# cvlab-stonybrook/s-volsdf

Hardware: AMD Instinct MI355X
Metric: rendered rays/sec (1024-ray batch, 128 samples) (higher is better)
Workload: dtype f32 (every product, forward and backward, as three fp16 MFMA products of two-piece fp16 operands with f32 accumulate; activation blocks hold both pieces: float32 accuracy class); 1 GPU; configs[1]: VolOpt.train_step (forward + MVS prior lookup + loss + backward + clip/guard/Adam), train mode, fast=1: 1024 rays/GPU x 128 coarse + 98 composited samples + 2048 eikonal points, 8x256 SDF MLP + 4x256 radiance MLP; mode=train, mlp_precision=fp16x2, launch=eager launches, rays_per_gpu=1024, rays_total=1024

## Files before the change

s-volsdf_amd/csrc/svs_sampler.hip:

```cpp
#include "svs_common.h"

namespace svs {
namespace sampler {

constexpr int kCap = 768;
constexpr int kMaxNew = 128;

struct Ctl {
  int conv_flag[8];
  int active[8];
  int final_round;
};

__device__ __forceinline__ float fma32(float a, float b, float c) { return __builtin_fmaf(a, b, c); }

__device__ __forceinline__ float linspace_at(float start, float end, int n, int i) {
  const float step = (end - start) / (float)(n - 1);
  return i < n / 2 ? fma32(step, (float)i, start) : fma32(-step, (float)(n - 1 - i), end);
}

__device__ __forceinline__ float wave_cumsum(const float* in, float* out, int m, int lane) {
  const int c = (m + 63) >> 6;
  const int lo = lane * c;
  const int hi = (lo + c < m) ? lo + c : m;
  double tot = 0.0;
  for (int j = lo; j < hi; ++j) tot = tot + (double)in[j];
  double scan = tot;
#pragma unroll
  for (int d = 1; d < 64; d <<= 1) {
    const double o = __shfl_up(scan, d);
    if (lane >= d) scan = scan + o;
  }
  double off = __shfl_up(scan, 1);
  if (lane == 0) off = 0.0;
  double acc = 0.0;
  float last = 0.0f;
  for (int j = lo; j < hi; ++j) {
    acc = acc + (double)in[j];
    last = (float)(off + acc);
    out[j] = last;
  }
  const int owner = (m - 1) / c;
  return __shfl(last, owner);
}

__device__ __forceinline__ float wave_max(float v) {
#pragma unroll
  for (int d = 32; d >= 1; d >>= 1) v = __builtin_fmaxf(v, __shfl_xor(v, d));
  return v;
}

struct RayLds {
  float z[kCap];
  float sdf[kCap];
  float dists[kCap];
  float dstar[kCap];
  float t0[kCap];
  float t1[kCap];
};

__device__ __forceinline__ void compute_dstar(RayLds& L, int n, int lane) {
  for (int i = lane; i < n - 1; i += 64) {
    const float a = L.z[i + 1] - L.z[i];
    const float d0 = L.sdf[i], d1 = L.sdf[i + 1];
    const float b = __builtin_fabsf(d0), c = __builtin_fabsf(d1);
    const float a2 = a * a, b2 = b * b, c2 = c * c;
    const bool first = (a2 + b2) <= c2;
    const bool second = (a2 + c2) <= b2;
    float ds = 0.0f;
    if (first) ds = b;
    if (second) ds = c;
    const float s = ((a + b) + c) / 2.0f;
    const float area = ((s * (s - a)) * (s - b)) * (s - c);
    if (!first && !second && ((b + c) - a > 0.0f)) ds = (2.0f * __builtin_sqrtf(area)) / a;
    const float sg0 = d0 > 0.0f ? 1.0f : (d0 < 0.0f ? -1.0f : 0.0f);
    const float sg1 = d1 > 0.0f ? 1.0f : (d1 < 0.0f ? -1.0f : 0.0f);
    const float same = (sg1 * sg0 == 1.0f) ? 1.0f : 0.0f;
    L.dists[i] = a;
    L.dstar[i] = same * ds;
  }
}

__device__ __forceinline__ float error_bound(RayLds& L, int n, float beta, int lane) {
  const float four_b2 = 4.0f * (beta * beta);
  for (int i = lane; i < n; i += 64) {
    L.t0[i] = i == 0 ? 0.0f : L.dists[i - 1] * laplace_density(L.sdf[i - 1], beta);
    if (i < n - 1) L.t1[i] = (sleef_expf(-L.dstar[i] / beta) * (L.dists[i] * L.dists[i])) / four_b2;
  }
  __syncthreads();
  wave_cumsum(L.t0, L.t0, n, lane);
  wave_cumsum(L.t1, L.t1, n - 1, lane);
  __syncthreads();
  float m = -__builtin_inff();
  bool has_nan = false;
  for (int i = lane; i < n - 1; i += 64) {
    const float e = sleef_expf(L.t1[i]);
    const float bo = ((e > 1.0e6f ? 1.0e6f : e) - 1.0f) * sleef_expf(-L.t0[i]);
    has_nan |= (bo != bo);
    m = __builtin_fmaxf(m, bo);
  }
  __syncthreads();
  m = wave_max(m);
  if (__any(has_nan)) m = __builtin_nanf("");
  return m;
}

struct InitArgs {
  const float* cam; int cam_stride; const float* dirs;
  int R;
  int n_eval;
  float near, far;
  int sphere_far;
  float sphere_radius;
  const float* jitter;
  float inv_4log;
  float* samples;
  float* beta;
  float* far_out;
  Ctl* ctl;
  int group_rays;
  int max_iters;
  int* err;
};

__global__ __launch_bounds__(64) void init_kernel(InitArgs a) {
  __shared__ float zs[kMaxNew];
  __shared__ float ds[kMaxNew];
  const int r = blockIdx.x, lane = threadIdx.x;
  if (r % a.group_rays == 0 && lane < 8) {
    Ctl* c = a.ctl + r / a.group_rays;
    c->conv_flag[lane] = 0;
    c->active[lane] = (lane == 0 && a.max_iters > 0) ? 1 : 0;
    if (lane == 0) c->final_round = -1;
  }
  float far = a.far;
  if (a.sphere_far) {
    const float* o = a.cam + (size_t)r * a.cam_stride;
    const float* d = a.dirs + 3 * (size_t)r;
    const float dot = (d[0] * o[0] + d[1] * o[1]) + d[2] * o[2];
    const float nrm = norm3(o[0], o[1], o[2]);
    const float under = dot * dot - (nrm * nrm - a.sphere_radius * a.sphere_radius);
    if (under <= 0.0f) { if (lane == 0) *a.err = 1; }
    far = __builtin_fmaxf(__builtin_sqrtf(under) - dot, 0.0f);
  }
  if (lane == 0) a.far_out[r] = far;
  const int n = a.n_eval;
  for (int i = lane; i < n; i += 64) {
    const float t = linspace_at(0.0f, 1.0f, n, i);
    zs[i] = a.near * (1.0f - t) + far * t;
  }
  __syncthreads();
  if (a.jitter) {
    float znew[(kMaxNew + 63) / 64];
    int k = 0;
    for (int i = lane; i < n; i += 64, ++k) {
      const float lower = i == 0 ? zs[0] : 0.5f * (zs[i] + zs[i - 1]);
      const float upper = i == n - 1 ? zs[n - 1] : 0.5f * (zs[i + 1] + zs[i]);
      znew[k] = lower + (upper - lower) * a.jitter[(size_t)r * n + i];
    }
    __syncthreads();
    k = 0;
    for (int i = lane; i < n; i += 64, ++k) zs[i] = znew[k];
    __syncthreads();
  }
  for (int i = lane; i < n; i += 64) {
    a.samples[(size_t)r * kMaxNew + i] = zs[i];
    if (i < n - 1) { const float d = zs[i + 1] - zs[i]; ds[i] = d * d; }
  }
  __syncthreads();
  const float tot = aten_row_sum(ds, n - 1, lane);
  if (lane == 0) a.beta[r] = __builtin_sqrtf(a.inv_4log * tot);
}

struct RoundArgs {
  int R, round, max_iters;
  int n_eval, n_final, n_extra;
  const float* beta_param; float beta_min;
  float eps; int beta_iters; float add_tiny;
  float near;
  const float* far;
  float* z;
  float* sdf;
  float* beta;
  float* samples;
  const float* samples_sdf;
  Ctl* ctl;
  int group_rays;
  const float* u_final;
  const int* extra_idx;
  const int* eik_idx;
  float* z_final;
  float* z_eik;
  int* dbg_samples_idx;
  int* dbg_inds;
  float* dbg_cdf;
  float* dbg_weights;
};

__global__ __launch_bounds__(64) void round_a_kernel(RoundArgs a) {
  __shared__ RayLds L;
  const int r = blockIdx.x, lane = threadIdx.x, i_round = a.round;
  Ctl* ctl = a.ctl + r / a.group_rays;
  if (!ctl->active[i_round]) return;
  const int n_old = a.n_eval * i_round, n_new = a.n_eval, n = n_old + n_new;
  float* zrow = a.z + (size_t)r * kCap;
  float* srow = a.sdf + (size_t)r * kCap;
  for (int i = lane; i < n_old; i += 64) { L.t0[i] = zrow[i]; L.t1[i] = srow[i]; }
  for (int i = lane; i < n_new; i += 64) {
    L.dists[i] = a.samples[(size_t)r * kMaxNew + i];
    L.dstar[i] = a.samples_sdf[(size_t)r * kMaxNew + i];
  }
  __syncthreads();
  for (int e = lane; e < n; e += 64) {
    int pos;
    float zv, sv;
    if (e < n_old) {
      zv = L.t0[e]; sv = L.t1[e];
      int cnt = 0;
      for (int k = 0; k < n_new; ++k) cnt += (L.dists[k] < zv) ? 1 : 0;
      pos = e + cnt;
    } else {
      const int j = e - n_old;
      zv = L.dists[j]; sv = L.dstar[j];
      int lo = 0, hi = n_old;
      while (lo < hi) { const int mid = (lo + hi) >> 1; if (L.t0[mid] <= zv) lo = mid + 1; else hi = mid; }
      int cnt = lo;
      for (int k = 0; k < n_new; ++k) {
        const float o = L.dists[k];
        cnt += (o < zv || (o == zv && k < j)) ? 1 : 0;
      }
      pos = cnt;
    }
    L.z[pos] = zv; L.sdf[pos] = sv;
    if (a.dbg_samples_idx) a.dbg_samples_idx[(size_t)r * kCap + pos] = e;
  }
  __syncthreads();
  for (int i = lane; i < n; i += 64) { zrow[i] = L.z[i]; srow[i] = L.sdf[i]; }
  compute_dstar(L, n, lane);
  __syncthreads();

  float beta = a.beta[r];
  const float beta0 = __builtin_fabsf(*a.beta_param) + a.beta_min;
  float err = error_bound(L, n, beta0, lane);
  if (err <= a.eps) beta = beta0;
  float bmin = beta0, bmax = beta;
  for (int it = 0; it < a.beta_iters; ++it) {
    const float mid = (bmin + bmax) / 2.0f;
    err = error_bound(L, n, mid, lane);
    if (err <= a.eps) bmax = mid;
    if (err > a.eps) bmin = mid;
  }
  beta = bmax;
  if (lane == 0) {
    a.beta[r] = beta;
    if (beta > beta0) atomicOr(&ctl->conv_flag[i_round], 1);
  }
}

__device__ __forceinline__ void finalize(const RoundArgs& a, RayLds& L, int r, int n, int ns, int lane) {
  const int m = ns + a.n_extra + 2;
  for (int i = lane; i < a.n_extra + 2; i += 64) {
    float v;
    if (i == 0) v = a.near;
    else if (i == 1) v = a.far[r];
    else {
      int idx;
      if (a.extra_idx) idx = a.extra_idx[i - 2];
      else idx = (int)linspace_at(0.0f, (float)(n - 1), a.n_extra, i - 2);
      v = L.z[idx];
    }
    L.t0[ns + i] = v;
  }
  __syncthreads();
  for (int e = lane; e < m; e += 64) {
    const float v = L.t0[e];
    int cnt = 0;
    for (int k = 0; k < m; ++k) { const float o = L.t0[k]; cnt += (o < v || (o == v && k < e)) ? 1 : 0; }
    L.t1[cnt] = v;
  }
  __syncthreads();
  for (int i = lane; i < m; i += 64) a.z_final[(size_t)r * m + i] = L.t1[i];
  if (lane == 0) a.z_eik[r] = L.t1[a.eik_idx ? a.eik_idx[r] : 0];
}

__global__ __launch_bounds__(64) void round_b_kernel(RoundArgs a) {
  __shared__ RayLds L;
  const int r = blockIdx.x, lane = threadIdx.x, i_round = a.round;
  Ctl* ctl = a.ctl + r / a.group_rays;
  if (!ctl->active[i_round]) return;
  const bool upsample = ctl->conv_flag[i_round] != 0 && (i_round + 1 < a.max_iters);
  if (r % a.group_rays == 0 && lane == 0) {
    ctl->active[i_round + 1] = upsample ? 1 : 0;
    if (!upsample) ctl->final_round = i_round;
  }
  const int n = a.n_eval * (i_round + 1);
  const float* zrow = a.z + (size_t)r * kCap;
  const float* srow = a.sdf + (size_t)r * kCap;
  for (int i = lane; i < n; i += 64) { L.z[i] = zrow[i]; L.sdf[i] = srow[i]; }
  __syncthreads();
  compute_dstar(L, n, lane);
  __syncthreads();
  const float beta = a.beta[r];
  for (int i = lane; i < n; i += 64) {
    L.t0[i] = i == 0 ? 0.0f : L.dists[i - 1] * laplace_density(L.sdf[i - 1], beta);
  }
  __syncthreads();
  wave_cumsum(L.t0, L.t0, n, lane);
  __syncthreads();
  for (int i = lane; i < n; i += 64) L.t0[i] = sleef_expf(-L.t0[i]);
  __syncthreads();
  const int N = upsample ? a.n_eval : a.n_final;
  if (upsample) {
    const float four_b2 = 4.0f * (beta * beta);
    for (int i = lane; i < n - 1; i += 64)
      L.t1[i] = (sleef_expf(-L.dstar[i] / beta) * (L.dists[i] * L.dists[i])) / four_b2;
    __syncthreads();
    wave_cumsum(L.t1, L.t1, n - 1, lane);
    __syncthreads();
    for (int i = lane; i < n - 1; i += 64) {
      const float e = sleef_expf(L.t1[i]);
      L.t1[i] = ((e > 1.0e6f ? 1.0e6f : e) - 1.0f) * L.t0[i] + a.add_tiny;
    }
  } else {
    for (int i = lane; i < n - 1; i += 64) {
      const float fe = L.dists[i] * laplace_density(L.sdf[i], beta);
      const float w = (1.0f - sleef_expf(-fe)) * L.t0[i];
      L.t1[i] = w + 1e-5f;
      if (a.dbg_weights) a.dbg_weights[(size_t)r * kCap + i] = w;
    }
  }
  __syncthreads();
  const float tot = aten_row_sum(L.t1, n - 1, lane);
  __syncthreads();
  for (int i = lane; i < n - 1; i += 64) L.t1[i] = L.t1[i] / tot;
  __syncthreads();
  wave_cumsum(L.t1, L.dstar, n - 1, lane);
  __syncthreads();
  for (int i = lane; i < n; i += 64) {
    const float c = i == 0 ? 0.0f : L.dstar[i - 1];
    L.t1[i] = c;
    if (a.dbg_cdf) a.dbg_cdf[(size_t)r * kCap + i] = c;
  }
  __syncthreads();
  for (int j = lane; j < N; j += 64) {
    float u;
    if (upsample || !a.u_final) u = linspace_at(0.0f, 1.0f, N, j);
    else u = a.u_final[(size_t)r * N + j];
    int lo = 0, hi = n;
    while (lo < hi) { const int mid = (lo + hi) >> 1; if (L.t1[mid] <= u) lo = mid + 1; else hi = mid; }
    const int inds = lo;
    const int below = inds - 1 > 0 ? inds - 1 : 0;
    const int above = inds < n - 1 ? inds : n - 1;
    const float cb = L.t1[below], ca = L.t1[above];
    const float zb = L.z[below], za = L.z[above];
    float denom = ca - cb;
    if (denom < 1e-5f) denom = 1.0f;
    const float t = (u - cb) / denom;
    L.dstar[j] = zb + t * (za - zb);
    if (a.dbg_inds) a.dbg_inds[(size_t)r * kMaxNew + j] = inds;
  }
  __syncthreads();
  if (upsample) {
    for (int j = lane; j < N; j += 64) a.samples[(size_t)r * kMaxNew + j] = L.dstar[j];
  } else {
    for (int j = lane; j < N; j += 64) L.t0[j] = L.dstar[j];
    __syncthreads();
    finalize(a, L, r, n, N, lane);
  }
}

__global__ __launch_bounds__(64) void finalize0_kernel(RoundArgs a) {
  __shared__ RayLds L;
  const int r = blockIdx.x, lane = threadIdx.x;
  for (int i = lane; i < a.n_eval; i += 64) {
    const float v = a.samples[(size_t)r * kMaxNew + i];
    L.z[i] = v; L.t0[i] = v;
  }
  __syncthreads();
  finalize(a, L, r, a.n_eval, a.n_eval, lane);
}

}
}

using namespace svs;
using namespace svs::sampler;

extern "C" {

size_t svs_sampler_ctl_bytes(int n_rays, int group_rays) {
  const int g = group_rays > 0 ? group_rays : (n_rays > 0 ? n_rays : 1);
  return (size_t)((n_rays + g - 1) / g) * sizeof(Ctl);
}
int svs_sampler_ctl_stride(void) { return (int)(sizeof(Ctl) / sizeof(int)); }
int svs_sampler_cap(void) { return kCap; }
int svs_sampler_max_new(void) { return kMaxNew; }

int svs_sampler_init(const float* cam, int cam_stride, const float* dirs, int n_rays, int n_eval, float near_, float far_,
                     int sphere_far, float sphere_radius, const float* jitter, float inv_4log, int max_iters,
                     float* samples, float* beta, float* far_out, void* ctl, int group_rays, int* err_flag,
                     void* hip_stream) {
  if (group_rays <= 0) group_rays = n_rays;
  if (!cam || !dirs || !samples || !beta || !far_out || !ctl || !err_flag || n_rays <= 0) {
    set_error("svs_sampler_init: null/invalid argument"); return SVS_EINVAL;
  }
  if (n_eval < 2 || n_eval > kMaxNew || max_iters < 0 || max_iters > 7 || n_eval * (max_iters > 0 ? max_iters : 1) > kCap) {
    set_error("svs_sampler_init: n_eval=%d max_iters=%d exceed the kernel limits (%d new / %d bins)", n_eval, max_iters, kMaxNew, kCap);
    return SVS_ESHAPE;
  }
  InitArgs a{cam, cam_stride, dirs, n_rays, n_eval, near_, far_, sphere_far, sphere_radius, jitter, inv_4log,
             samples, beta, far_out, (Ctl*)ctl, group_rays, max_iters, err_flag};
  init_kernel<<<n_rays, 64, 0, (hipStream_t)hip_stream>>>(a);
  return check_launch("svs_sampler_init");
}

int svs_sampler_round(int phase, int n_rays, int round, int max_iters, int n_eval, int n_final, int n_extra,
                      const float* beta_param, float beta_min, float eps, int beta_iters, float add_tiny, float near_,
                      const float* far_,
                      float* z, float* sdf, float* beta, float* samples, const float* samples_sdf, void* ctl,
                      int group_rays, const float* u_final, const int* extra_idx, const int* eik_idx, float* z_final, float* z_eik,
                      int* dbg_samples_idx, int* dbg_inds, float* dbg_cdf, float* dbg_weights, void* hip_stream) {
  if (!beta_param || !far_ || !z || !sdf || !beta || !samples || !ctl || !z_final || !z_eik || n_rays <= 0 || round < 0 || round > 6) {
    set_error("svs_sampler_round: null/invalid argument"); return SVS_EINVAL;
  }
  if (group_rays <= 0) group_rays = n_rays;
  if (n_final > kMaxNew || n_final + n_extra + 2 > kCap || n_eval + n_extra + 2 > kCap) {
    set_error("svs_sampler_round: sample counts exceed kernel limits"); return SVS_ESHAPE;
  }
  RoundArgs a{n_rays, round, max_iters, n_eval, n_final, n_extra, beta_param, beta_min, eps, beta_iters, add_tiny, near_, far_,
              z, sdf, beta, samples, samples_sdf, (Ctl*)ctl, group_rays, u_final, extra_idx, eik_idx, z_final, z_eik,
              dbg_samples_idx, dbg_inds, dbg_cdf, dbg_weights};
  hipStream_t s = (hipStream_t)hip_stream;
  if (phase == 0) {
    if (!samples_sdf) { set_error("svs_sampler_round: round A needs samples_sdf"); return SVS_EINVAL; }
    round_a_kernel<<<n_rays, 64, 0, s>>>(a);
  } else if (phase == 1) {
    round_b_kernel<<<n_rays, 64, 0, s>>>(a);
  } else {
    finalize0_kernel<<<n_rays, 64, 0, s>>>(a);
  }
  return check_launch("svs_sampler_round");
}

__global__ void selftest_exp_kernel(const float* x, float* y_exp, float* y_expm1, int n) {
  const int i = blockIdx.x * blockDim.x + threadIdx.x;
  if (i < n) { y_exp[i] = sleef_expf(x[i]); y_expm1[i] = sleef_expm1f(x[i]); }
}
__global__ void selftest_arith_kernel(const float* a, const float* b, float* q, float* s, int n) {
  const int i = blockIdx.x * blockDim.x + threadIdx.x;
  if (i < n) { q[i] = a[i] / b[i]; s[i] = __builtin_sqrtf(__builtin_fabsf(a[i])); }
}
__global__ __launch_bounds__(64) void selftest_cumsum_kernel(const float* x, float* y, float* tot, int m) {
  __shared__ float buf[kCap];
  const int lane = threadIdx.x;
  for (int i = lane; i < m; i += 64) buf[i] = x[(size_t)blockIdx.x * m + i];
  __syncthreads();
  const float t = wave_cumsum(buf, buf, m, lane);
  __syncthreads();
  for (int i = lane; i < m; i += 64) y[(size_t)blockIdx.x * m + i] = buf[i];
  if (lane == 0) tot[blockIdx.x] = t;
}

__global__ __launch_bounds__(64) void selftest_rowsum_kernel(const float* x, float* tot, int m) {
  extern __shared__ float rowbuf[];
  const int lane = threadIdx.x;
  for (int i = lane; i < m; i += 64) rowbuf[i] = x[(size_t)blockIdx.x * m + i];
  __syncthreads();
  const float t = aten_row_sum(rowbuf, m, lane);
  if (lane == 0) tot[blockIdx.x] = t;
}

int svs_selftest_rowsum(const float* x, float* tot, int rows, int m, void* hip_stream) {
  if (m < 1 || m > 16000) { set_error("svs_selftest_rowsum: m out of range (1..16000)"); return SVS_ESHAPE; }
  selftest_rowsum_kernel<<<rows, 64, (size_t)m * sizeof(float), (hipStream_t)hip_stream>>>(x, tot, m);
  return check_launch("svs_selftest_rowsum");
}
int svs_selftest_exp(const float* x, float* y_exp, float* y_expm1, int n, void* hip_stream) {
  selftest_exp_kernel<<<(n + 255) / 256, 256, 0, (hipStream_t)hip_stream>>>(x, y_exp, y_expm1, n);
  return check_launch("svs_selftest_exp");
}
int svs_selftest_arith(const float* a, const float* b, float* q, float* s, int n, void* hip_stream) {
  selftest_arith_kernel<<<(n + 255) / 256, 256, 0, (hipStream_t)hip_stream>>>(a, b, q, s, n);
  return check_launch("svs_selftest_arith");
}
int svs_selftest_cumsum(const float* x, float* y, float* tot, int rows, int m, void* hip_stream) {
  if (m < 1 || m > kCap) { set_error("svs_selftest_cumsum: m out of range"); return SVS_ESHAPE; }
  selftest_cumsum_kernel<<<rows, 64, 0, (hipStream_t)hip_stream>>>(x, y, tot, m);
  return check_launch("svs_selftest_cumsum");
}

}
```

s-volsdf_amd/svs_hip/ops.py:

```python
import ctypes
import os

import torch

from . import lib as _lib


def _ptr(t):
    if t is None:
        return None
    assert t.is_cuda and t.is_contiguous(), "device-resident contiguous tensors only"
    return t.data_ptr()


_raw_stream = getattr(torch._C, "_cuda_getCurrentRawStream", None)


def _stream():
    if _raw_stream is not None:
        return _raw_stream(torch.cuda.current_device())
    return torch.cuda.current_stream().cuda_stream


def _f32(t):
# ... 355 lines not shown
        cam, dirs, z = _f32(cam).reshape(3), _f32(dirs), _f32(z)
        R, S = z.shape
        dev = z.device
    V = len(views)
    ver = lambda t: (id(t), getattr(t, "_version", 0))
    key = tuple((ver(v["K"]), ver(v["c2w"]), v["cost"].data_ptr(), v["cost"].shape,
                 (v["z_mvs"].data_ptr(), v["z_mvs"].shape) if "z_mvs" in v else (v["z_near"].data_ptr(), v["z_far"].data_ptr()))
                for v in views)
    hit = _LOOKUP_CONSTS.get(key)
    if hit is None:
        vp = (ctypes.c_float * (17 * V))()
        dims = (ctypes.c_int * (3 * V))()
        keep, cost_p, near_p, far_p = [], [], [], []
        copied = False
        for j, v in enumerate(views):
            K, c2w = _host_f32(v["K"]), _host_f32(v["c2w"])
            vals = [K[0, 0], K[1, 1], K[0, 2], K[1, 2], K[0, 1]] + [c2w[i, k] for i in range(3) for k in range(4)]
            for k, x in enumerate(vals):
                vp[17 * j + k] = float(x)
            cost = _f32(v["cost"]).reshape(v["cost"].shape[-3:])
            if "z_mvs" in v:
                zm = v["z_mvs"].reshape(v["z_mvs"].shape[-3:])
                zn, zf = _f32(zm[0]), _f32(zm[-1])
                copied = copied or zn.data_ptr() != zm[0].data_ptr() or zf.data_ptr() != zm[-1].data_ptr()
            else:
                zn, zf = _f32(v["z_near"]), _f32(v["z_far"])
                copied = copied or zn.data_ptr() != v["z_near"].data_ptr() or zf.data_ptr() != v["z_far"].data_ptr()
            keep += [cost, zn, zf, v["K"], v["c2w"], v["cost"], v.get("z_mvs"), v.get("z_near"), v.get("z_far")]
            copied = copied or cost.data_ptr() != v["cost"].data_ptr()
            cost_p.append(cost); near_p.append(zn); far_p.append(zf)
            dims[3 * j], dims[3 * j + 1], dims[3 * j + 2] = cost.shape
        if len(_LOOKUP_CONSTS) >= 4:
            _LOOKUP_CONSTS.clear()
        hit = (vp, dims, _ptr_array(cost_p), _ptr_array(near_p), _ptr_array(far_p), keep)
        if not copied:
            _LOOKUP_CONSTS[key] = hit
    vp, dims, cost_arr, near_arr, far_arr, _ = hit
    pj = torch.empty(R, S, device=dev)
    pi = torch.empty(R, S, device=dev)
    valid = torch.empty(R, S, dtype=torch.uint8, device=dev)
    _lib.check(L.svs_cost_lookup(_ptr(xyz), _ptr(cam), _ptr(dirs), _ptr(z), S, R * S, V, int(same_view),
                                 int(bool(inverse_depth)), float(img_res[1]), float(img_res[0]), vp,
                                 cost_arr, near_arr, far_arr, dims, _ptr(pj), _ptr(pi),
                                 _ptr(valid), _ptr(same_view_dev), _stream()), "svs_cost_lookup")
    return pj, pi, valid.view(torch.bool)


def loss_fwd_bwd(rgb_values, rgb_target, weights, depth_values, grad_theta=None, pi=None, pj=None, *, rgb_weight=1.0,
                 eikonal_weight=0.1, mvs_weight=0.0, sparse_weight=0.0, gce=1.0, confi=0.0, annealed=False,
                 anneal_sparse=0.0, norm=None, anneal_dev=None, grad_theta_out=None):
    L = _lib.load()
    rgb_values, rgb_target = _f32(rgb_values).reshape(-1, 3), _f32(rgb_target).reshape(-1, 3)
    weights, depth_values = _f32(weights), _f32(depth_values).reshape(-1)
    R, S = weights.shape
    dev = weights.device
    gt = _f32(grad_theta) if grad_theta is not None else None
    n_eik = gt.shape[0] if gt is not None else 0
    pi_, pj_ = (_f32(pi), _f32(pj)) if pi is not None else (None, None)
    losses = torch.empty(5, device=dev)
    d_rgb = torch.empty(R, 3, device=dev)
    d_gt = None
    if n_eik:
        ok = (grad_theta_out is not None and grad_theta_out.is_cuda and grad_theta_out.dtype == torch.float32
              and tuple(grad_theta_out.shape) == (n_eik, 3) and grad_theta_out.is_contiguous())
        d_gt = grad_theta_out if ok else torch.empty(n_eik, 3, device=dev)
    d_w = torch.empty(R, S, device=dev)
    d_dep = torch.empty(R, 1, device=dev)
    ws = torch.empty(L.svs_loss_workspace_bytes(R, n_eik) // 8, dtype=torch.float64, device=dev)
    _lib.check(L.svs_loss(R, S, n_eik, _ptr(rgb_values), _ptr(rgb_target), _ptr(gt), _ptr(weights), _ptr(pi_), _ptr(pj_),
                          _ptr(depth_values), float(rgb_weight), float(eikonal_weight), float(mvs_weight),
                          float(sparse_weight), float(gce), float(confi), int(bool(annealed)), float(anneal_sparse),
                          int(norm[0]) if norm else 0, int(norm[1]) if norm else 0, _ptr(losses), _ptr(d_rgb), _ptr(d_gt), _ptr(d_w), _ptr(d_dep), _ptr(ws),
                          _ptr(anneal_dev), _stream()), "svs_loss")
    return losses, dict(rgb_values=d_rgb, grad_theta=d_gt, weights=d_w, depth_values=d_dep)


class SamplerWorkspace:

    def __init__(self, R, device, group_rays=None):
        L = _lib.load()
        self.R = R
        self.group_rays = int(group_rays) if group_rays else R
        self.cap, self.max_new = L.svs_sampler_cap(), L.svs_sampler_max_new()
        f = lambda *s: torch.empty(*s, device=device)
        self.z, self.sdf = f(R, self.cap), f(R, self.cap)
        self.beta, self.far = f(R), f(R)
        self.samples, self.samples_sdf = f(R, self.max_new), f(R, self.max_new)
        self.ctl = torch.zeros(L.svs_sampler_ctl_bytes(R, self.group_rays) // 4, dtype=torch.int32, device=device)
        self.ctl_stride = L.svs_sampler_ctl_stride()
        self.err = torch.zeros(1, dtype=torch.int32, device=device)


def sample_rays(packed, cam, dirs, beta_param, *, beta_min=1e-4, near, scene_bounding_sphere, sphere_scale, sdf_clamp_radius,
                N_samples=64, N_samples_eval=128, N_samples_extra=32, eps=0.1, beta_iters=10, max_total_iters=5,
                fast=-1, training=False, inverse_sphere_bg=False, add_tiny=0.0, inv_4log=None, rng=None,
                workspace=None, debug=None, sdf_override=None):
    L = _lib.load()
    cam, dirs = _f32(cam), _f32(dirs)
    R = dirs.shape[0]
    dev = dirs.device
    ws = workspace or SamplerWorkspace(R, dev)
    assert ws.R == R
    rng = rng or {}
    if not torch.is_tensor(beta_param):
        beta_param = torch.tensor(float(beta_param), device=dev)
    beta_param = _f32(beta_param).reshape(1)
    max_iters = fast if fast >= 0 else max_total_iters
    if training and max_iters > 1 and "perm" in rng:
        raise NotImplementedError("train-mode extras for more than one round need the bin count on the host")
    if inv_4log is None:
        inv_4log = float(1.0 / (4.0 * torch.log(torch.tensor(eps + 1.0))))
    cam_stride = 0 if cam.numel() == 3 else 3
    far = 2.0 * scene_bounding_sphere
    jitter = _f32(rng["jitter"]) if training and "jitter" in rng else None
    _lib.check(L.svs_sampler_init(_ptr(cam), cam_stride, _ptr(dirs), R, N_samples_eval, float(near), float(far),
                                  int(inverse_sphere_bg), float(scene_bounding_sphere), _ptr(jitter), float(inv_4log),
                                  max_iters, _ptr(ws.samples), _ptr(ws.beta), _ptr(ws.far), _ptr(ws.ctl), ws.group_rays,
                                  _ptr(ws.err), _stream()), "svs_sampler_init")
    n_out = (N_samples if max_iters > 0 else N_samples_eval) + N_samples_extra + 2
    z_final = torch.empty(R, n_out, device=dev)
    z_eik = torch.empty(R, 1, device=dev)
    u_final = _f32(rng["u"]) if training and "u" in rng else None
    extra_idx = rng["perm"].to(torch.int32).contiguous() if training and "perm" in rng else None
    eik_idx = rng["eik_idx"].to(torch.int32).contiguous() if training and "eik_idx" in rng else None

    def call(phase, i, dbg):
        _lib.check(L.svs_sampler_round(phase, R, i, max_iters, N_samples_eval, N_samples, N_samples_extra, _ptr(beta_param),
                                       float(beta_min), float(eps), beta_iters, float(add_tiny), float(near), _ptr(ws.far), _ptr(ws.z),
                                       _ptr(ws.sdf), _ptr(ws.beta), _ptr(ws.samples), _ptr(ws.samples_sdf), _ptr(ws.ctl),
                                       ws.group_rays, _ptr(u_final), _ptr(extra_idx), _ptr(eik_idx), _ptr(z_final), _ptr(z_eik),
                                       _ptr(dbg.get("samples_idx")), _ptr(dbg.get("inds")), _ptr(dbg.get("cdf")),
                                       _ptr(dbg.get("weights")), _stream()), "svs_sampler_round")

    if max_iters == 0:
        call(2, 0, {})
        return z_final, z_eik
    src = PointSource(cam=cam, dirs=dirs, z=ws.samples[:, :N_samples_eval]) if N_samples_eval == ws.max_new else None
    for i in range(max_iters):
        dbg = {}
        if debug is not None:
            dbg = dict(samples_idx=torch.full((R, ws.cap), -1, dtype=torch.int32, device=dev),
                       inds=torch.full((R, ws.max_new), -1, dtype=torch.int32, device=dev),
                       cdf=torch.zeros(R, ws.cap, device=dev), weights=torch.zeros(R, ws.cap, device=dev))
            debug.setdefault("rounds", []).append(dbg)
        if sdf_override is not None:
            if i < len(sdf_override):
                ws.samples_sdf[:, :N_samples_eval].copy_(sdf_override[i])
        else:
            if src is None:
                raise NotImplementedError("N_samples_eval must equal the kernel's row stride (128)")
            gate = ws.ctl.data_ptr() + 4 * (8 + i)
            sdf_vals(packed, src, sdf_clamp_radius, sphere_scale, out=ws.samples_sdf, gate=gate,
                     gate_points=ws.group_rays * N_samples_eval, gate_stride=ws.ctl_stride)
        call(0, i, dbg)
        call(1, i, dbg)
        if debug is not None:
            dbg["z"] = ws.z.clone(); dbg["sdf"] = ws.sdf.clone(); dbg["beta"] = ws.beta.clone()
            dbg["samples"] = ws.samples.clone(); dbg["ctl"] = ws.ctl.clone()
    return z_final, z_eik
```

s-volsdf_amd/svs_hip/trainer.py:

```python
import ctypes

import os

import torch

from . import lib as _lib
from . import ops
from .ops import _ptr, _stream


class FlatParams:

    def __init__(self, params):
        self.params = [p for p in params]
        dev = self.params[0].device
        n = sum(p.numel() for p in self.params)
        self.flat = torch.empty(n, device=dev)
        self.grad = torch.zeros(n, device=dev)
        off = 0
        for p in self.params:
            k = p.numel()
            self.flat[off:off + k].copy_(p.data.reshape(-1))
            p.data = self.flat[off:off + k].view(p.shape)
            p.grad = self.grad[off:off + k].view(p.shape)
            off += k
        self.n = n

    def views(self, buf):
        out, off = [], 0
        for p in self.params:
            out.append(buf[off:off + p.numel()].view(p.shape))
            off += p.numel()
        return out


class FusedAdam:

    def __init__(self, params, lr=5e-4, betas=(0.9, 0.999), eps=1e-8, max_norm=1.0):
        self.fp = params if isinstance(params, FlatParams) else FlatParams(list(params))
        self.lr, self.betas, self.eps, self.max_norm = lr, betas, eps, max_norm
        dev = self.fp.flat.device
        self.exp_avg = torch.zeros_like(self.fp.flat)
        self.exp_avg_sq = torch.zeros_like(self.fp.flat)
        L = _lib.load()
        self.ws = torch.empty(L.svs_adam_workspace_bytes() // 4, dtype=torch.int32, device=dev)
        self.info = torch.zeros(2, device=dev)
        self.step_count = 0
        self.step_dev = None

    def zero_grad(self, set_to_none=False):
        self.fp.grad.zero_()

    def step(self):
        L = _lib.load()
        self.step_count += 1
        _lib.check(L.svs_clip_guard_adam(_ptr(self.fp.flat), _ptr(self.fp.grad), _ptr(self.exp_avg), _ptr(self.exp_avg_sq),
                                         self.fp.n, self.step_count, _ptr(self.step_dev) if self.step_dev is not None else None,
                                         float(self.max_norm), float(self.lr), float(self.betas[0]), float(self.betas[1]),
                                         float(self.eps), _ptr(self.ws), _ptr(self.info), _stream()), "svs_clip_guard_adam")

    def state_dict(self):
        return {"step": self.step_count, "exp_avg": self.exp_avg, "exp_avg_sq": self.exp_avg_sq}

    def load_state_dict(self, sd):
        self.step_count = int(sd["step"])
        self.exp_avg.copy_(sd["exp_avg"]); self.exp_avg_sq.copy_(sd["exp_avg_sq"])


def shard_rays(uv, rank, world):
    R = uv.shape[1]
    if R % world:
        raise ValueError(f"{R} rays do not shard over {world} ranks")
    k = R // world
    return uv[:, rank * k:(rank + 1) * k]


def allreduce_flat_grad(flat_grad, world):
    import torch.distributed as dist
    if world > 1 or (dist.is_available() and dist.is_initialized()):
        dist.all_reduce(flat_grad, op=dist.ReduceOp.SUM)
    return flat_grad


def data_parallel(world):
    import torch.distributed as dist
    return world > 1 or (dist.is_available() and dist.is_initialized())


def grad_buckets(n_sdf, n):
    return [(n_sdf, n), (0, n_sdf)]


def allreduce_range(flat_grad, lo, hi, async_op=False):
    import torch.distributed as dist
    return dist.all_reduce(flat_grad[lo:hi], op=dist.ReduceOp.SUM, async_op=async_op)


_DP_BUCKETS = os.environ.get("SVS_DP_BUCKETS", "1") == "1"


class _GroupedOutputs(dict):

    def __init__(self, results):
        super().__init__()
        self._parts = [r[1] for r in results]

    def __missing__(self, key):
        vals = [p[key] for p in self._parts]
        self[key] = torch.cat(vals, 0) if torch.is_tensor(vals[0]) and vals[0].dim() > 0 else vals[0]
        return self[key]

    def __contains__(self, key):
        return key in self._parts[0]

    def keys(self):
        return self._parts[0].keys()


class _ValidRays(dict):

    def __init__(self, outputs, n_valid, n_padded):
        super().__init__()
        self._o, self._v, self._p = outputs, n_valid, n_padded

    def __missing__(self, key):
        t = self._o[key]
        if torch.is_tensor(t) and t.dim() > 0:
            if key == "grad_theta" and t.shape[0] == 2 * self._p:
                t = torch.cat([t[:self._v], t[self._p:self._p + self._v]], 0)
            elif t.shape[0] == self._p:
                t = t[:self._v]
            elif t.shape[0] % self._p == 0 and t.shape[0] > self._p:
                t = t.reshape(self._p, -1, *t.shape[1:])[:self._v].reshape(-1, *t.shape[1:])
        self[key] = t
        return t

    def __contains__(self, key):
        return key in self._o

    def keys(self):
        return self._o.keys()


class _GroupedLosses(dict):

    def __init__(self, results):
        super().__init__()
        self._parts = [r[0] for r in results]

    def __missing__(self, key):
        vals = [p[key] for p in self._parts]
        self[key] = torch.stack(vals).sum(0) if torch.is_tensor(vals[0]) else sum(vals)
        return self[key]

    def __contains__(self, key):
        return key in self._parts[0]

    def keys(self):
        return self._parts[0].keys()

    def items(self):
# ... 450 lines not shown
                    comm.wait_event(ev)
                finalize(sc.accum, sdf_p, rgb_p, out=self.grad_out, nets=(1,))
                if self.is_bg:
                    sc.bg_bwd.finalize(bg_sdf_wb, bg_rgb_wb, out=self.bg_grad_out)
                if len(groups) > 1:
                    torch.sum(sc.d_beta[:len(groups)], dim=0, keepdim=True, out=self.beta_grad.view(1))
                lo, hi = self._buckets[0]
                self._early_work = allreduce_range(self.fp.grad, lo, hi, async_op=True)
        for ev in joins:
            main.wait_event(ev)
        finalize(sc.accum, sdf_p, rgb_p, out=self.grad_out, nets=(0,) if early else (0, 1))
        if self.is_bg and not early:
            sc.bg_bwd.finalize(bg_sdf_wb, bg_rgb_wb, out=self.bg_grad_out)
        if len(groups) == 1 or early:
            pass
        else:
            torch.sum(sc.d_beta[:len(groups)], dim=0, keepdim=True, out=self.beta_grad.view(1))
        return results, holds

    def _capture_key(self, model_input, mvs, fast):
        R = model_input["uv"].shape[1]
        mk = None
        if mvs is not None:
            def view_key(v):
                ptrs = tuple((int(v[k].data_ptr()), tuple(v[k].shape)) for k in ("cost", "z_mvs") if torch.is_tensor(v.get(k)))
                cams = []
                for k in sorted(v):
                    if k in ("cost", "z_mvs"):
                        continue
                    x = v[k]
                    if torch.is_tensor(x):
                        cams.append((k, int(x.data_ptr()), x._version, tuple(x.shape)))
                    else:
                        cams.append((k, repr(x)))
                return ptrs, tuple(cams)
            mk = (len(mvs["views"]), tuple(mvs["img_res"]), bool(mvs.get("inverse_depth", False)),
                  tuple(view_key(v) for v in mvs["views"]))
        return (R, getattr(self, "_n_valid", R), tuple(self._groups_for(R)), fast, mk, str(self.fp.flat.device), self.graph)

    def _upload(self, cs, model_input, ground_truth, mvs):
        st = cs.static
        dev = self.fp.flat.device
        annealed, anneal_sparse = self.loss.anneal_state()
        target = ground_truth["rgb_smooth"] if annealed else ground_truth["rgb"]
        origin = {k: model_input[k] for k in ("uv", "intrinsics", "pose")}
        origin["target"] = target
        pieces = [(k, model_input[k]) for k in ("uv", "intrinsics", "pose")] + [("target", target.reshape(-1, 3))]
        if "_all" not in st:
            off = 4
            st["_layout"] = {}
            for k, src in pieces:
                st["_layout"][k] = (off, tuple(src.shape))
                off += (src.numel() + 3) // 4 * 4
            st["_all"] = torch.zeros(off, dtype=torch.float32, device=dev)
            st["_ring"] = [dict(pin=torch.zeros(off, dtype=torch.float32).pin_memory(), ev=None) for _ in range(4)]
            st["_i"] = 0
            for k, (o, shape) in st["_layout"].items():
                n = 1
                for d in shape:
                    n *= d
                st[k] = st["_all"][o:o + n].view(shape)
            st["anneal"] = st["_all"][0:2]
            st["same_view"] = st["_all"][2:3].view(torch.int32)
            st["rng"] = {}
        slot = st["_ring"][st["_i"] % 4]
        st["_i"] += 1
        if slot["ev"] is not None:
            slot["ev"].synchronize()
        pin = slot["pin"]
        pin[0] = 1.0 if annealed else 0.0
        pin[1] = float(anneal_sparse)
        pin[2:3].view(torch.int32)[0] = int(mvs["same_view"]) if mvs is not None else -1
        on_device, host = [], False
        seen = st.setdefault("_seen", {})
        for k, src in pieces:
            o, shape = st["_layout"][k]
            if tuple(src.shape) != shape:
                raise ValueError(f"captured step: input {k} changed shape {shape} -> {tuple(src.shape)}")
            if src.is_cuda:
                tag = (origin[k], origin[k]._version)
                old = seen.get(k)
                if old is None or old[0] is not tag[0] or old[1] != tag[1]:
                    on_device.append((k, src, tag))
            else:
                pin[o:o + src.numel()].copy_(src.reshape(-1))
                host = True
                seen.pop(k, None)
        head = (float(pin[0]), float(pin[1]), int(pin[2:3].view(torch.int32)[0]))
        if host:
            if any(src.is_cuda for _, src in pieces):
                on_device = [(k, src, (origin[k], origin[k]._version)) for k, src in pieces if src.is_cuda]
            ops.stage_in(st["_all"], pin)
        elif st.get("_head") != head:
            ops.stage_in(st["_all"][:4], pin[:4])
        if host or st.get("_head") != head:
            slot["ev"] = torch.cuda.Event()
            slot["ev"].record()
            st["_head"] = head
        for k, src, tag in on_device:
            st[k].copy_(src, non_blocking=True)
            seen[k] = tag
        n_valid, n_pad = getattr(self, "_n_valid", model_input["uv"].shape[1]), model_input["uv"].shape[1]
        m = self.model
        sharded = self.world > 1 and self.shard_draws
        if sharded or n_valid < n_pad:
            if sharded:
                drawn = m.slice_rng(m.draw_train_rng(n_valid * self.world, dev), self.rank * n_valid, (self.rank + 1) * n_valid)
            else:
                drawn = m.draw_train_rng(n_valid, dev)
            if n_valid < n_pad:
                from volsdf.model.network import pad_rng
                drawn = pad_rng(drawn, n_pad)
            for k, v in drawn.items():
                if k.startswith("_"):
                    continue
                if k not in st["rng"]:
                    st["rng"][k] = torch.empty_like(v)
                st["rng"][k].copy_(v, non_blocking=True)
        else:
            m.draw_train_rng(n_pad, dev, out=st["rng"])

    def _step_captured(self, model_input, ground_truth, mvs, fast):
        key = self._capture_key(model_input, mvs, fast)
        cs = self._captured.get(key)
        if cs is None:
            if len(self._captured) >= 4:
                self._evicted = self._captured.pop(next(iter(self._captured)))
            cs = self._captured[key] = _CapturedStep()
        cs.calls += 1
        if cs.calls == 1:
            return None
        m = self.model
        self._upload(cs, model_input, ground_truth, mvs)
        self._draws_done()
        if cs.graph is None:
            st = cs.static
            cs.scratch = _Scratch(self.fp.flat.device, self.is_bg)
            inp = dict(model_input)
            inp.update(uv=st["uv"], intrinsics=st["intrinsics"], pose=st["pose"])
            gt = {"rgb": st["target"], "rgb_smooth": st["target"]}
            dyn = dict(same_view=st["same_view"], anneal=st["anneal"])
            if getattr(self, "_capture_stream", None) is None:
                self._capture_stream = torch.cuda.Stream(device=self.fp.flat.device)
            cap = self._capture_stream
            cap.wait_stream(torch.cuda.current_stream())
            with torch.cuda.stream(cap):
                self._device_step(cs.scratch, inp, gt, mvs, fast, st["rng"], dyn, serial=self.graph == "linear")
            torch.cuda.current_stream().wait_stream(cap)
            m.invalidate_packed()
            plan_mode = self.graph in ("plan", "auto")
            graph = torch.cuda.CUDAGraph(keep_graph=True) if plan_mode else torch.cuda.CUDAGraph()
            if self._graph_pool is None:
                self._graph_pool = torch.cuda.graph_pool_handle()
            import gc
            gc_was_on = gc.isenabled()
            gc.disable()
            try:
                with torch.cuda.graph(graph, pool=self._graph_pool, stream=cap, capture_error_mode="thread_local"):
                    cs.result, cs.hold = self._device_step(cs.scratch, inp, gt, mvs, fast, st["rng"], dyn,
                                                           serial=self.graph == "linear")
            finally:
                if gc_was_on:
                    gc.enable()
            cs.graph = graph
            if plan_mode:
                sc = cs.scratch
                side = ([sc.prep] + list(sc.sides) + [b._side for b in sc.bwd] + list(getattr(m, "_bg_streams", {}).values())
                        + list(sc._bg_streams.values()))
                try:
                    cs.plan = _LaunchPlan(graph, [x for x in side if x is not None])
                except _lib.SvsError as e:
                    if self.graph != "auto":
                        raise
                    import warnings
                    warnings.warn(f"launch plan refused, this configuration replays its hipGraph instead: {e}")
                    cs.plan = None
                    graph.instantiate()
                    if os.environ.get("SVS_PLAN_DEBUG") == "1":
                        import sys
                        print(f"launch plan refused: {e}", file=sys.stderr)
                if cs.plan is not None and os.environ.get("SVS_PLAN_DEBUG") == "1":
                    import sys
                    print(cs.plan.info, file=sys.stderr)
                    print(cs.plan.describe(), file=sys.stderr)
        if cs.plan is not None:
            cs.plan.run()
        else:
            cs.graph.replay()
        return cs.result


def loss_norm(n_rays_local, world):
    return n_rays_local * world, 2 * n_rays_local * world
```

Before: 291,700 rays/s.

## Parallelize sampler beta bisection across waves and fuse final round A/B

Round A of the error-bounded sampler now launches several waves per ray and evaluates multiple bisection midpoints speculatively in parallel, one per wave, walking a binary tree of candidates so each step advances several bisection levels. On the last round, a fused phase runs the round B resampling/finalize tail in wave 0 of the same kernel, with wave-level syncs in place of block barriers, which removes a kernel launch and an LDS reload. This trades extra total arithmetic and dynamic LDS (lower occupancy) for less serial latency in the bisection. It also adds a GC-idle wait before graph capture, which is a robustness fix.

```diff
diff --git a/s-volsdf_amd/csrc/svs_sampler.hip b/s-volsdf_amd/csrc/svs_sampler.hip
--- a/s-volsdf_amd/csrc/svs_sampler.hip
+++ b/s-volsdf_amd/csrc/svs_sampler.hip
@@ -59,8 +59,28 @@
   float t1[kCap];
 };
 
-__device__ __forceinline__ void compute_dstar(RayLds& L, int n, int lane) {
-  for (int i = lane; i < n - 1; i += 64) {
+struct RayView {
+  float* z;
+  float* sdf;
+  float* dists;
+  float* dstar;
+  float* t0;
+  float* t1;
+};
+
+struct BlockSync {
+  static __device__ __forceinline__ void sync() { __syncthreads(); }
+};
+struct WaveSync {
+  static __device__ __forceinline__ void sync() {
+    asm volatile("s_waitcnt lgkmcnt(0)" ::: "memory");
+    __builtin_amdgcn_wave_barrier();
+  }
+};
+
+template <class LDS>
+__device__ __forceinline__ void compute_dstar(LDS& L, int n, int tid, int nt = 64) {
+  for (int i = tid; i < n - 1; i += nt) {
     const float a = L.z[i + 1] - L.z[i];
     const float d0 = L.sdf[i], d1 = L.sdf[i + 1];
     const float b = __builtin_fabsf(d0), c = __builtin_fabsf(d1);
@@ -81,25 +101,25 @@
   }
 }
 
-__device__ __forceinline__ float error_bound(RayLds& L, int n, float beta, int lane) {
+__device__ __forceinline__ float error_bound(const RayView& L, float* t0, float* t1, int n, float beta, int lane) {
   const float four_b2 = 4.0f * (beta * beta);
   for (int i = lane; i < n; i += 64) {
-    L.t0[i] = i == 0 ? 0.0f : L.dists[i - 1] * laplace_density(L.sdf[i - 1], beta);
-    if (i < n - 1) L.t1[i] = (sleef_expf(-L.dstar[i] / beta) * (L.dists[i] * L.dists[i])) / four_b2;
-  }
-  __syncthreads();
-  wave_cumsum(L.t0, L.t0, n, lane);
-  wave_cumsum(L.t1, L.t1, n - 1, lane);
-  __syncthreads();
+    t0[i] = i == 0 ? 0.0f : L.dists[i - 1] * laplace_density(L.sdf[i - 1], beta);
+    if (i < n - 1) t1[i] = (sleef_expf(-L.dstar[i] / beta) * (L.dists[i] * L.dists[i])) / four_b2;
+  }
+  WaveSync::sync();
+  wave_cumsum(t0, t0, n, lane);
+  wave_cumsum(t1, t1, n - 1, lane);
+  WaveSync::sync();
   float m = -__builtin_inff();
   bool has_nan = false;
   for (int i = lane; i < n - 1; i += 64) {
-    const float e = sleef_expf(L.t1[i]);
-    const float bo = ((e > 1.0e6f ? 1.0e6f : e) - 1.0f) * sleef_expf(-L.t0[i]);
+    const float e = sleef_expf(t1[i]);
+    const float bo = ((e > 1.0e6f ? 1.0e6f : e) - 1.0f) * sleef_expf(-t0[i]);
     has_nan |= (bo != bo);
     m = __builtin_fmaxf(m, bo);
   }
-  __syncthreads();
+  WaveSync::sync();
   m = wave_max(m);
   if (__any(has_nan)) m = __builtin_nanf("");
   return m;
@@ -197,67 +217,8 @@
   float* dbg_weights;
 };
 
-__global__ __launch_bounds__(64) void round_a_kernel(RoundArgs a) {
-  __shared__ RayLds L;
-  const int r = blockIdx.x, lane = threadIdx.x, i_round = a.round;
-  Ctl* ctl = a.ctl + r / a.group_rays;
-  if (!ctl->active[i_round]) return;
-  const int n_old = a.n_eval * i_round, n_new = a.n_eval, n = n_old + n_new;
-  float* zrow = a.z + (size_t)r * kCap;
-  float* srow = a.sdf + (size_t)r * kCap;
-  for (int i = lane; i < n_old; i += 64) { L.t0[i] = zrow[i]; L.t1[i] = srow[i]; }
-  for (int i = lane; i < n_new; i += 64) {
-    L.dists[i] = a.samples[(size_t)r * kMaxNew + i];
-    L.dstar[i] = a.samples_sdf[(size_t)r * kMaxNew + i];
-  }
-  __syncthreads();
-  for (int e = lane; e < n; e += 64) {
-    int pos;
-    float zv, sv;
-    if (e < n_old) {
-      zv = L.t0[e]; sv = L.t1[e];
-      int cnt = 0;
-      for (int k = 0; k < n_new; ++k) cnt += (L.dists[k] < zv) ? 1 : 0;
-      pos = e + cnt;
-    } else {
-      const int j = e - n_old;
-      zv = L.dists[j]; sv = L.dstar[j];
-      int lo = 0, hi = n_old;
-      while (lo < hi) { const int mid = (lo + hi) >> 1; if (L.t0[mid] <= zv) lo = mid + 1; else hi = mid; }
-      int cnt = lo;
-      for (int k = 0; k < n_new; ++k) {
-        const float o = L.dists[k];
-        cnt += (o < zv || (o == zv && k < j)) ? 1 : 0;
-      }
-      pos = cnt;
-    }
-    L.z[pos] = zv; L.sdf[pos] = sv;
-    if (a.dbg_samples_idx) a.dbg_samples_idx[(size_t)r * kCap + pos] = e;
-  }
-  __syncthreads();
-  for (int i = lane; i < n; i += 64) { zrow[i] = L.z[i]; srow[i] = L.sdf[i]; }
-  compute_dstar(L, n, lane);
-  __syncthreads();
-
-  float beta = a.beta[r];
-  const float beta0 = __builtin_fabsf(*a.beta_param) + a.beta_min;
-  float err = error_bound(L, n, beta0, lane);
-  if (err <= a.eps) beta = beta0;
-  float bmin = beta0, bmax = beta;
-  for (int it = 0; it < a.beta_iters; ++it) {
-    const float mid = (bmin + bmax) / 2.0f;
-    err = error_bound(L, n, mid, lane);
-    if (err <= a.eps) bmax = mid;
-    if (err > a.eps) bmin = mid;
-  }
-  beta = bmax;
-  if (lane == 0) {
-    a.beta[r] = beta;
-    if (beta > beta0) atomicOr(&ctl->conv_flag[i_round], 1);
-  }
-}
-
-__device__ __forceinline__ void finalize(const RoundArgs& a, RayLds& L, int r, int n, int ns, int lane) {
+template <class Sync, class LDS>
+__device__ __forceinline__ void finalize(const RoundArgs& a, LDS& L, int r, int n, int ns, int lane) {
   const int m = ns + a.n_extra + 2;
   for (int i = lane; i < a.n_extra + 2; i += 64) {
     float v;
@@ -271,52 +232,36 @@
     }
     L.t0[ns + i] = v;
   }
-  __syncthreads();
+  Sync::sync();
   for (int e = lane; e < m; e += 64) {
     const float v = L.t0[e];
     int cnt = 0;
     for (int k = 0; k < m; ++k) { const float o = L.t0[k]; cnt += (o < v || (o == v && k < e)) ? 1 : 0; }
     L.t1[cnt] = v;
   }
-  __syncthreads();
+  Sync::sync();
   for (int i = lane; i < m; i += 64) a.z_final[(size_t)r * m + i] = L.t1[i];
   if (lane == 0) a.z_eik[r] = L.t1[a.eik_idx ? a.eik_idx[r] : 0];
 }
 
-__global__ __launch_bounds__(64) void round_b_kernel(RoundArgs a) {
-  __shared__ RayLds L;
-  const int r = blockIdx.x, lane = threadIdx.x, i_round = a.round;
-  Ctl* ctl = a.ctl + r / a.group_rays;
-  if (!ctl->active[i_round]) return;
-  const bool upsample = ctl->conv_flag[i_round] != 0 && (i_round + 1 < a.max_iters);
-  if (r % a.group_rays == 0 && lane == 0) {
-    ctl->active[i_round + 1] = upsample ? 1 : 0;
-    if (!upsample) ctl->final_round = i_round;
-  }
-  const int n = a.n_eval * (i_round + 1);
-  const float* zrow = a.z + (size_t)r * kCap;
-  const float* srow = a.sdf + (size_t)r * kCap;
-  for (int i = lane; i < n; i += 64) { L.z[i] = zrow[i]; L.sdf[i] = srow[i]; }
-  __syncthreads();
-  compute_dstar(L, n, lane);
-  __syncthreads();
-  const float beta = a.beta[r];
+template <class Sync, class LDS>
+__device__ __forceinline__ void round_b_tail(const RoundArgs& a, LDS& L, int r, int n, bool upsample, float beta, int lane) {
   for (int i = lane; i < n; i += 64) {
     L.t0[i] = i == 0 ? 0.0f : L.dists[i - 1] * laplace_density(L.sdf[i - 1], beta);
   }
-  __syncthreads();
+  Sync::sync();
   wave_cumsum(L.t0, L.t0, n, lane);
-  __syncthreads();
+  Sync::sync();
   for (int i = lane; i < n; i += 64) L.t0[i] = sleef_expf(-L.t0[i]);
-  __syncthreads();
+  Sync::sync();
   const int N = upsample ? a.n_eval : a.n_final;
   if (upsample) {
     const float four_b2 = 4.0f * (beta * beta);
     for (int i = lane; i < n - 1; i += 64)
       L.t1[i] = (sleef_expf(-L.dstar[i] / beta) * (L.dists[i] * L.dists[i])) / four_b2;
-    __syncthreads();
+    Sync::sync();
     wave_cumsum(L.t1, L.t1, n - 1, lane);
-    __syncthreads();
+    Sync::sync();
     for (int i = lane; i < n - 1; i += 64) {
       const float e = sleef_expf(L.t1[i]);
       L.t1[i] = ((e > 1.0e6f ? 1.0e6f : e) - 1.0f) * L.t0[i] + a.add_tiny;
@@ -329,19 +274,19 @@
       if (a.dbg_weights) a.dbg_weights[(size_t)r * kCap + i] = w;
     }
   }
-  __syncthreads();
+  Sync::sync();
   const float tot = aten_row_sum(L.t1, n - 1, lane);
-  __syncthreads();
+  Sync::sync();
   for (int i = lane; i < n - 1; i += 64) L.t1[i] = L.t1[i] / tot;
-  __syncthreads();
+  Sync::sync();
   wave_cumsum(L.t1, L.dstar, n - 1, lane);
-  __syncthreads();
+  Sync::sync();
   for (int i = lane; i < n; i += 64) {
     const float c = i == 0 ? 0.0f : L.dstar[i - 1];
     L.t1[i] = c;
     if (a.dbg_cdf) a.dbg_cdf[(size_t)r * kCap + i] = c;
   }
-  __syncthreads();
+  Sync::sync();
   for (int j = lane; j < N; j += 64) {
     float u;
     if (upsample || !a.u_final) u = linspace_at(0.0f, 1.0f, N, j);
@@ -359,14 +304,158 @@
     L.dstar[j] = zb + t * (za - zb);
     if (a.dbg_inds) a.dbg_inds[(size_t)r * kMaxNew + j] = inds;
   }
-  __syncthreads();
+  Sync::sync();
   if (upsample) {
     for (int j = lane; j < N; j += 64) a.samples[(size_t)r * kMaxNew + j] = L.dstar[j];
   } else {
     for (int j = lane; j < N; j += 64) L.t0[j] = L.dstar[j];
+    Sync::sync();
+    finalize<Sync>(a, L, r, n, N, lane);
+  }
+}
+
+template <int LV>
+__device__ __forceinline__ float beta_search(const RayView& L, float* scratch, int rs, int n, float beta_in, float beta0,
+                                             float eps, int iters, int wave, int lane) {
+  constexpr int C = (1 << LV) - 1;
+  float* t0 = scratch + (size_t)wave * 2 * rs;
+  float* t1 = t0 + rs;
+  auto err_of = [&](int w) { return scratch[(size_t)w * 2 * rs + rs + n - 1]; };
+  const int id = wave + 1, depth = 31 - __builtin_clz(id);
+  float bmin = beta0, bmax = beta_in;
+  bool first = true;
+  int done = 0;
+  for (;;) {
+    const int lv = iters - done < LV ? iters - done : LV;
+    float e = 0.0f;
+    if (first && wave == C) {
+      e = error_bound(L, t0, t1, n, beta0, lane);
+    } else if (wave < C && depth < lv) {
+      float lo = bmin, hi = bmax;
+      for (int j = depth - 1; j >= 0; --j) {
+        const float mid = (lo + hi) / 2.0f;
+        if ((id >> j) & 1) lo = mid; else hi = mid;
+      }
+      e = error_bound(L, t0, t1, n, (lo + hi) / 2.0f, lane);
+    }
+    if (lane == 0) t1[n - 1] = e;
     __syncthreads();
-    finalize(a, L, r, n, N, lane);
-  }
+    bool walk = true;
+    if (first) {
+      first = false;
+      if (err_of(C) <= eps) {
+        bmax = beta0;
+        if ((beta0 + beta0) / 2.0f == beta0) return bmax;
+        walk = false;
+      }
+    }
+    if (walk) {
+      int k = 1;
+      for (int l = 0; l < lv; ++l) {
+        const float mid = (bmin + bmax) / 2.0f;
+        const float el = err_of(k - 1);
+        if (el <= eps) { bmax = mid; k = 2 * k; }
+        else if (el > eps) { bmin = mid; k = 2 * k + 1; }
+        else return bmax;
+      }
+      done += lv;
+    }
+    if (done >= iters) return bmax;
+    __syncthreads();
+  }
+}
+
+__host__ __device__ constexpr int row_stride(int n, int m) { return m > n ? m : n; }
+__host__ __device__ constexpr size_t lds_floats(int lv, int n, int m) { return (size_t)row_stride(n, m) * (4 + (2 << lv)); }
+constexpr size_t kLdsQuarter = 160 * 1024 / 4;
+static_assert(lds_floats(2, kCap, kCap) * sizeof(float) <= kLdsQuarter, "the 3-candidate round A must fit 4 workgroups per CU");
+
+template <int LV, bool FUSED>
+__global__ __launch_bounds__(64 << LV, LV == 3 ? 8 : 4) void round_a_kernel(RoundArgs a, int rs) {
+  extern __shared__ float lds[];
+  constexpr int NT = 64 << LV;
+  const int r = blockIdx.x, tid = threadIdx.x, lane = tid & 63, i_round = a.round;
+  const int wave = __builtin_amdgcn_readfirstlane(tid >> 6);
+  Ctl* ctl = a.ctl + r / a.group_rays;
+  if (!ctl->active[i_round]) return;
+  const int n_old = a.n_eval * i_round, n_new = a.n_eval, n = n_old + n_new;
+  RayView L{lds, lds + rs, lds + 2 * rs, lds + 3 * rs, nullptr, nullptr};
+  float* scratch = lds + 4 * rs;
+  float* zrow = a.z + (size_t)r * kCap;
+  float* srow = a.sdf + (size_t)r * kCap;
+  float* oz = scratch;
+  float* os = scratch + rs;
+  for (int i = tid; i < n_old; i += NT) { oz[i] = zrow[i]; os[i] = srow[i]; }
+  for (int i = tid; i < n_new; i += NT) {
+    L.dists[i] = a.samples[(size_t)r * kMaxNew + i];
+    L.dstar[i] = a.samples_sdf[(size_t)r * kMaxNew + i];
+  }
+  __syncthreads();
+  for (int e = tid; e < n; e += NT) {
+    int pos;
+    float zv, sv;
+    if (e < n_old) {
+      zv = oz[e]; sv = os[e];
+      int cnt = 0;
+      for (int k = 0; k < n_new; ++k) cnt += (L.dists[k] < zv) ? 1 : 0;
+      pos = e + cnt;
+    } else {
+      const int j = e - n_old;
+      zv = L.dists[j]; sv = L.dstar[j];
+      int lo = 0, hi = n_old;
+      while (lo < hi) { const int mid = (lo + hi) >> 1; if (oz[mid] <= zv) lo = mid + 1; else hi = mid; }
+      int cnt = lo;
+      for (int k = 0; k < n_new; ++k) {
+        const float o = L.dists[k];
+        cnt += (o < zv || (o == zv && k < j)) ? 1 : 0;
+      }
+      pos = cnt;
+    }
+    L.z[pos] = zv; L.sdf[pos] = sv;
+    if (a.dbg_samples_idx) a.dbg_samples_idx[(size_t)r * kCap + pos] = e;
+  }
+  __syncthreads();
+  for (int i = tid; i < n; i += NT) { zrow[i] = L.z[i]; srow[i] = L.sdf[i]; }
+  compute_dstar(L, n, tid, NT);
+  __syncthreads();
+
+  const float beta0 = __builtin_fabsf(*a.beta_param) + a.beta_min;
+  const float beta = beta_search<LV>(L, scratch, rs, n, a.beta[r], beta0, a.eps, a.beta_iters, wave, lane);
+  if (tid == 0) {
+    a.beta[r] = beta;
+    if (beta > beta0) atomicOr(&ctl->conv_flag[i_round], 1);
+  }
+  if constexpr (FUSED) {
+    __syncthreads();
+    if (wave != 0) return;
+    if (r % a.group_rays == 0 && lane == 0) {
+      ctl->active[i_round + 1] = 0;
+      ctl->final_round = i_round;
+    }
+    L.t0 = scratch;
+    L.t1 = scratch + rs;
+    round_b_tail<WaveSync>(a, L, r, n, false, beta, lane);
+  }
+}
+
+__global__ __launch_bounds__(64) void round_b_kernel(RoundArgs a) {
+  __shared__ RayLds L;
+  const int r = blockIdx.x, lane = threadIdx.x, i_round = a.round;
+  Ctl* ctl = a.ctl + r / a.group_rays;
+  if (!ctl->active[i_round]) return;
+  const bool upsample = ctl->conv_flag[i_round] != 0 && (i_round + 1 < a.max_iters);
+  if (r % a.group_rays == 0 && lane == 0) {
+    ctl->active[i_round + 1] = upsample ? 1 : 0;
+    if (!upsample) ctl->final_round = i_round;
+  }
+  const int n = a.n_eval * (i_round + 1);
+  const float* zrow = a.z + (size_t)r * kCap;
+  const float* srow = a.sdf + (size_t)r * kCap;
+  for (int i = lane; i < n; i += 64) { L.z[i] = zrow[i]; L.sdf[i] = srow[i]; }
+  __syncthreads();
+  compute_dstar(L, n, lane);
+  __syncthreads();
+  round_b_tail<BlockSync>(a, L, r, n, upsample, a.beta[r], lane);
 }
 
 __global__ __launch_bounds__(64) void finalize0_kernel(RoundArgs a) {
@@ -377,7 +466,12 @@
     L.z[i] = v; L.t0[i] = v;
   }
   __syncthreads();
-  finalize(a, L, r, a.n_eval, a.n_eval, lane);
+  finalize<BlockSync>(a, L, r, a.n_eval, a.n_eval, lane);
+}
+
+template <int LV, bool FUSED>
+static void launch_round_a(const RoundArgs& a, int n, int m, hipStream_t s) {
+  round_a_kernel<LV, FUSED><<<a.R, 64 << LV, lds_floats(LV, n, m) * sizeof(float), s>>>(a, row_stride(n, m));
 }
 
 }
@@ -423,6 +517,7 @@
   if (!beta_param || !far_ || !z || !sdf || !beta || !samples || !ctl || !z_final || !z_eik || n_rays <= 0 || round < 0 || round > 6) {
     set_error("svs_sampler_round: null/invalid argument"); return SVS_EINVAL;
   }
+  if (phase < 0 || phase > 3) { set_error("svs_sampler_round: phase %d is none of 0..3", phase); return SVS_EINVAL; }
   if (group_rays <= 0) group_rays = n_rays;
   if (n_final > kMaxNew || n_final + n_extra + 2 > kCap || n_eval + n_extra + 2 > kCap) {
     set_error("svs_sampler_round: sample counts exceed kernel limits"); return SVS_ESHAPE;
@@ -431,9 +526,21 @@
               z, sdf, beta, samples, samples_sdf, (Ctl*)ctl, group_rays, u_final, extra_idx, eik_idx, z_final, z_eik,
               dbg_samples_idx, dbg_inds, dbg_cdf, dbg_weights};
   hipStream_t s = (hipStream_t)hip_stream;
-  if (phase == 0) {
+  if (phase == 0 || phase == 3) {
     if (!samples_sdf) { set_error("svs_sampler_round: round A needs samples_sdf"); return SVS_EINVAL; }
-    round_a_kernel<<<n_rays, 64, 0, s>>>(a);
+    const int n = n_eval * (round + 1);
+    if (n_eval < 2 || n_eval > kMaxNew || n > kCap) {
+      set_error("svs_sampler_round: n_eval=%d round=%d exceed the kernel limits (%d new / %d bins)", n_eval, round, kMaxNew, kCap);
+      return SVS_ESHAPE;
+    }
+    if (phase == 3 && round + 1 < max_iters) {
+      set_error("svs_sampler_round: phase 3 is for the last round (round %d of %d may up-sample)", round, max_iters);
+      return SVS_EINVAL;
+    }
+    const int m = phase == 3 ? n_final + n_extra + 2 : 0;
+    const bool seven = lds_floats(3, n, m) * sizeof(float) <= kLdsQuarter;
+    if (phase == 0) { if (seven) launch_round_a<3, false>(a, n, m, s); else launch_round_a<2, false>(a, n, m, s); }
+    else { if (seven) launch_round_a<3, true>(a, n, m, s); else launch_round_a<2, true>(a, n, m, s); }
   } else if (phase == 1) {
     round_b_kernel<<<n_rays, 64, 0, s>>>(a);
   } else {
diff --git a/s-volsdf_amd/svs_hip/ops.py b/s-volsdf_amd/svs_hip/ops.py
--- a/s-volsdf_amd/svs_hip/ops.py
+++ b/s-volsdf_amd/svs_hip/ops.py
@@ -531,8 +531,11 @@
             gate = ws.ctl.data_ptr() + 4 * (8 + i)
             sdf_vals(packed, src, sdf_clamp_radius, sphere_scale, out=ws.samples_sdf, gate=gate,
                      gate_points=ws.group_rays * N_samples_eval, gate_stride=ws.ctl_stride)
-        call(0, i, dbg)
-        call(1, i, dbg)
+        if i + 1 >= max_iters and debug is None:
+            call(3, i, dbg)
+        else:
+            call(0, i, dbg)
+            call(1, i, dbg)
         if debug is not None:
             dbg["z"] = ws.z.clone(); dbg["sdf"] = ws.sdf.clone(); dbg["beta"] = ws.beta.clone()
             dbg["samples"] = ws.samples.clone(); dbg["ctl"] = ws.ctl.clone()
diff --git a/s-volsdf_amd/svs_hip/trainer.py b/s-volsdf_amd/svs_hip/trainer.py
--- a/s-volsdf_amd/svs_hip/trainer.py
+++ b/s-volsdf_amd/svs_hip/trainer.py
@@ -1,12 +1,26 @@
 import ctypes
-
+import gc
 import os
+import threading
 
 import torch
 
 from . import lib as _lib
 from . import ops
 from .ops import _ptr, _stream
+
+_GC_IDLE = threading.Event()
+_GC_IDLE.set()
+
+
+def _gc_watch(phase, info):
+    if phase == "start":
+        _GC_IDLE.clear()
+    else:
+        _GC_IDLE.set()
+
+
+gc.callbacks.append(_gc_watch)
 
 
 class FlatParams:
@@ -763,9 +777,9 @@
             graph = torch.cuda.CUDAGraph(keep_graph=True) if plan_mode else torch.cuda.CUDAGraph()
             if self._graph_pool is None:
                 self._graph_pool = torch.cuda.graph_pool_handle()
-            import gc
             gc_was_on = gc.isenabled()
             gc.disable()
+            _GC_IDLE.wait()
             try:
                 with torch.cuda.graph(graph, pool=self._graph_pool, stream=cap, capture_error_mode="thread_local"):
                     cs.result, cs.hold = self._device_step(cs.scratch, inp, gt, mvs, fast, st["rng"], dyn,
```

Result: no change. 291,400 rays/s (-0.1%).
